# jeffreyyu0602/quantized-training

Hardware: AMD Instinct MI355X
Metric: quantized_elements_per_sec (higher is better)
Workload: dtype bf16; 1 GPU; llama-2-7b-shaped LLaMA (32 layers, hidden 4096, random init) WikiText-style window eval B=1 S=1024 stride 512, fake-quant activation=e4m3 weight=e4m3, --quantize_forward gemm (weights re-quantized every forward); route=eager, parallelism=dp1 (windows round-robin, metric all_gather only), launch=hipGraph replay, valid=True

## Files before the change

### quantized-training_amd/csrc/qt_attention_fp8.hip

```cpp
#include <hip/hip_runtime.h>
#include <stdint.h>
#include <stdlib.h>

#include "../../include/qt_hip.h"
#include "qt_device.h"
#include "qt_attention_split.h"
#include "qt_value_codes.h"
#include "qt_formats.h"

namespace {

typedef int v8i __attribute__((ext_vector_type(8)));

constexpr int kUnit = 127;

struct AttnArgs {
    const uint8_t *q8, *k8, *vt8;
    const uint16_t *mask;
    long msb, msh, msq;
    const int *row_live;
    long lsb, lsh, lsq;
    int mask_simple;
    uint16_t *out;
    int H, Sq, Sk;
// ... 18 lines not shown
        o = __builtin_amdgcn_cvt_scalef32_pk_fp8_bf16(o, __builtin_bit_cast(v2bf, p1), 1.0f, true);
    }
    return __builtin_bit_cast(uint32_t, o);
}

template <int F, int D, int MODE>
__device__ __forceinline__ void score_half(const uint8_t *blk, int t0, const v8i &qf, int f_lo, int f_hi, float scaling, float (*ev)[4], float &mx,
                                           const uint16_t *mrow, int key0, int my_live, int tiles) {
    uint2 m[4];
    if (MODE == 2) {
#pragma unroll
        for (int j = 0; j < 4; ++j) m[j] = *(const uint2 *)(mrow + key0 + j * 16);
    }
    u32x4 klo[4], khi[4];
#pragma unroll
    for (int j = 0; j < 4; ++j) {
        if (MODE == 1 && j >= tiles) continue;
        klo[j] = *(const u32x4 *)(blk + (t0 + j) * (16 * D) + f_lo);
        if (D == 128) khi[j] = *(const u32x4 *)(blk + (t0 + j) * (16 * D) + f_hi);
        else khi[j] = u32x4{0u, 0u, 0u, 0u};
    }
    v4f s[4];
#pragma unroll
    for (int j = 0; j < 4; ++j) {
        if (MODE == 1 && j >= tiles) continue;
        const v8i kf = {(int)klo[j].x, (int)klo[j].y, (int)klo[j].z, (int)klo[j].w, (int)khi[j].x, (int)khi[j].y, (int)khi[j].z, (int)khi[j].w};
        s[j] = __builtin_amdgcn_mfma_scale_f32_16x16x128_f8f6f4(kf, qf, v4f{0.f, 0.f, 0.f, 0.f}, F, F, 0, kUnit, 0, kUnit);
    }
    __builtin_amdgcn_sched_barrier(0);
#pragma unroll
    for (int j = 0; j < 4; ++j) {
        if (MODE == 1 && j >= tiles) {
            ev[j][0] = ev[j][1] = ev[j][2] = ev[j][3] = -INFINITY;
            continue;
        }
        uint32_t w0 = pack_bf16x2(s[j][0], s[j][1]), w1 = pack_bf16x2(s[j][2], s[j][3]);
        w0 = pack_bf16x2(bf_lo(w0) * scaling, bf_hi(w0) * scaling);
        w1 = pack_bf16x2(bf_lo(w1) * scaling, bf_hi(w1) * scaling);
        if (MODE == 2) {
            w0 = pack_bf16x2(bf_lo(w0) + bf_lo(m[j].x), bf_hi(w0) + bf_hi(m[j].x));
            w1 = pack_bf16x2(bf_lo(w1) + bf_lo(m[j].y), bf_hi(w1) + bf_hi(m[j].y));
        }
        float v[4] = {bf_lo(w0), bf_hi(w0), bf_lo(w1), bf_hi(w1)};
        if (MODE == 1) {
            const int left = my_live - (key0 + j * 16);
#pragma unroll
            for (int e = 0; e < 4; ++e) v[e] = (e < left || v[e] != v[e]) ? v[e] : -3.3895313892515355e38f;
        }
        ev[j][0] = v[0]; ev[j][1] = v[1]; ev[j][2] = v[2]; ev[j][3] = v[3];
        mx = max3(mx, v[0], v[1]);
        mx = max3(mx, v[2], v[3]);
    }
}

template <int F, int D, int MB>
__global__ __launch_bounds__(512, (MB == 4 && D == 64) ? 4 : 1) void attention_fp8_split_kernel(AttnArgs a) {
    constexpr int kBuf = kBlock * D;
    constexpr int kPieces = D / 32;
    extern __shared__ __attribute__((aligned(16))) uint8_t lds[];
    const int t = threadIdx.x, l = t & 63, w = __builtin_amdgcn_readfirstlane(t >> 6);
    const int r = l & 15, g = l >> 4, grp = w >> 2, wq = w & 3;
    const int bh = blockIdx.x, b = bh / a.H, h = bh % a.H;
    const int nkb = a.Sk / kBlock, nqb = (a.Sq + 63) / 64;
    const int qb = nqb - 1 - (int)blockIdx.y;
    const int q0 = qb * 64;
    const int qrow = q0 + wq * 16 + r, qc = min(qrow, a.Sq - 1);
    int nlive, wmax, wmin, my_live;
    split_row_extents(a, b, h, q0, qc, l, nkb, nlive, wmax, wmin, my_live);
    const int niter = (nlive + 1) / 2;
    const bool simple = a.mask && a.row_live && (a.mask_simple || (a.mask_irregular && *a.mask_irregular == 0)), full = a.mask && !simple;
    if (!simple) wmin = a.Sk;
    if (!simple && !a.row_live) wmax = a.Sk;
    const uint32_t l0 = lds_addr(lds);
    const uint8_t *kp[kPieces], *vp[kPieces];
#pragma unroll
    for (int i = 0; i < kPieces; ++i) {
        const int piece = (w * kPieces + i) % (D / 8);
        if (D == 128) {
            const int row = piece * 8 + (l >> 3), slot = l & 7, sw = ((slot ^ ((row >> 1) & 7)) << 4);
            kp[i] = a.k8 + ((long)bh * a.Sk + row) * D + sw;
        } else {
            const int r16 = l >> 2, row = piece * 16 + r16, sw = (((l & 3) ^ (((r16 >> 3) & 1) << 1)) << 4);
            kp[i] = a.k8 + ((long)bh * a.Sk + row) * D + sw;
        }
        const int vrow = piece * 8 + (l >> 3), vslot = l & 7, vsw = ((vslot ^ ((vrow >> 1) & 7)) << 4);
        vp[i] = a.vt8 + ((long)bh * D + vrow) * a.Sk + vsw;
    }
    auto issue_k = [&](int it) {
#pragma unroll
        for (int i = 0; i < kPieces; ++i) {
            const int piece = w * kPieces + i, kb = min(2 * it + piece / (D / 8), nkb - 1);
            dma16(kp[i] + (long)kb * kBuf, l0 + (2 * it) * kBuf + piece * 1024);
        }
    };
    auto issue_v = [&](int it) {
#pragma unroll
        for (int i = 0; i < kPieces; ++i) {
            const int piece = w * kPieces + i, kb = min(2 * it + piece / (D / 8), nkb - 1);
            dma16(vp[i] + (long)kb * kBlock, l0 + (2 * it) * kBuf + piece * 1024);
        }
    };
    auto wait_pair = [&](int it) {
        if (it + 1 < niter) asm volatile("s_waitcnt vmcnt(%0)" ::"n"(kPieces) : "memory");
        else asm volatile("s_waitcnt vmcnt(0)" ::: "memory");
        __builtin_amdgcn_s_barrier();
    };
// ... 68 lines not shown
    float sum = sum2[0] + sum2[1];
    sum += __shfl_xor(sum, 16, 64);
    sum += __shfl_xor(sum, 32, 64);
    if (g == 0) stat[128 + grp * 64 + wq * 16 + r] = sum;
    __syncthreads();
    const float inv = 1.0f / (stat[128 + wq * 16 + r] + stat[128 + 64 + wq * 16 + r]);
    constexpr int kDT = D / 16;
    v4f acc[kDT];
#pragma unroll
    for (int i = 0; i < kDT; ++i) acc[i] = v4f{0.f, 0.f, 0.f, 0.f};
#pragma unroll
    for (int it = 0; it < kIter; ++it) {
        if (it < niter) {
            wait_pair(it);
            if (it + 2 < niter) issue_v(it + 2);
            const bool live0 = tiles_of(2 * it) != 0, live1 = tiles_of(2 * it + 1) != 0;
            if (live0 | live1) {
                const uint8_t *blk = lds + (2 * it) * kBuf + f_v;
                u32x4 vlo[kDT], vhi[kDT];
#pragma unroll
                for (int dt = 0; dt < kDT / 2; ++dt) {
                    vlo[dt] = *(const u32x4 *)(blk + dt * 2048);
                    vhi[dt] = *(const u32x4 *)(blk + kBuf + dt * 2048);
                }
                uint32_t pd[8];
#pragma unroll
                for (int c = 0; c < 2; ++c) {
                    if (c == 0 ? live0 : live1) {
#pragma unroll
                        for (int j = 4 * c; j < 4 * c + 4; ++j) {
                            const float *v = e[it][j];
                            const uint32_t p0 = pack_bf16x2(v[0] * inv, v[1] * inv), p1 = pack_bf16x2(v[2] * inv, v[3] * inv);
                            pd[j] = prob_codes<F == 1>(p0, p1);
                        }
                    } else {
                        pd[4 * c] = pd[4 * c + 1] = pd[4 * c + 2] = pd[4 * c + 3] = 0;
                    }
                }
                const v8i pf = {(int)pd[0], (int)pd[1], (int)pd[2], (int)pd[3], (int)pd[4], (int)pd[5], (int)pd[6], (int)pd[7]};
#pragma unroll
                for (int dt = kDT / 2; dt < kDT; ++dt) {
                    vlo[dt] = *(const u32x4 *)(blk + dt * 2048);
                    vhi[dt] = *(const u32x4 *)(blk + kBuf + dt * 2048);
                }
                __builtin_amdgcn_sched_barrier(0);
#pragma unroll
                for (int dt = 0; dt < kDT; ++dt) {
                    const v8i vf = {(int)vlo[dt].x, (int)vlo[dt].y, (int)vlo[dt].z, (int)vlo[dt].w, (int)vhi[dt].x, (int)vhi[dt].y, (int)vhi[dt].z, (int)vhi[dt].w};
                    acc[dt] = __builtin_amdgcn_mfma_scale_f32_16x16x128_f8f6f4(vf, pf, acc[dt], F, F, 0, kUnit, 0, kUnit);
                }
            }
        }
    }
    const int prow = wq * 16 + r;
    split_park_partials(lds, acc, grp, prow, g);
    if (grp == 0 && qrow < a.Sq) {
#pragma unroll
        for (int dt = 0; dt < kDT; ++dt) {
            const float4 o = split_partial_sums<kDT>(lds, prow, dt, g);
            acc[dt][0] += o.x; acc[dt][1] += o.y; acc[dt][2] += o.z; acc[dt][3] += o.w;
        }
        const long o0 = (((long)b * a.Sq + qrow) * a.H + h) * D + 4 * g;
        uint16_t *orow = a.out + o0;
        if (a.out8) {
            const bool oe5 = a.out_fmt.p0 == 2;
#pragma unroll
            for (int dt = 0; dt < kDT; dt += 2) {
                uint32_t o[4] = {pack_bf16x2(acc[dt][0], acc[dt][1]), pack_bf16x2(acc[dt][2], acc[dt][3]),
                                 pack_bf16x2(acc[dt + 1][0], acc[dt + 1][1]), pack_bf16x2(acc[dt + 1][2], acc[dt + 1][3])};
                const uint2 codes = oe5 ? fq8_hw_vec8<true>(o, a.out_fmt) : fq8_hw_vec8<false>(o, a.out_fmt);
                *(uint2 *)(orow + dt * 16) = uint2{o[0], o[1]};
                *(uint2 *)(orow + dt * 16 + 16) = uint2{o[2], o[3]};
                *(uint32_t *)(a.out8 + o0 + dt * 16) = codes.x;
                *(uint32_t *)(a.out8 + o0 + dt * 16 + 16) = codes.y;
            }
        } else {
#pragma unroll
            for (int dt = 0; dt < kDT; ++dt)
                *(uint2 *)(orow + dt * 16) = uint2{pack_bf16x2(acc[dt][0], acc[dt][1]), pack_bf16x2(acc[dt][2], acc[dt][3])};
        }
    }
}

template <bool E5M2, int D>
__global__ __launch_bounds__(256) void value_codes_t_kernel(const uint16_t *v, uint8_t *vt8, int H, long Sk, long sb, long sh, long sk,
                                                            qt_format fmt) {
    __shared__ __attribute__((aligned(16))) uint8_t tile[D * kBlock];
    value_codes_block<E5M2, D>(tile, v, vt8, (int)blockIdx.x, (long)blockIdx.y, H, Sk, sb, sh, sk, fmt);
}

template <int F, int D, int MB>
int launch_split_mb(const AttnArgs &a, long BH, int nqb, hipStream_t st) {
    constexpr int kLds = MB * kBlock * D + 2 * 2 * 64 * 4;
    static_assert(MB * kBlock * D >= 64 * (D + 4) * 4, "the partial sums of the second wave group reuse the block buffers");
    if (qt_allow_lds<attention_fp8_split_kernel<F, D, MB>>(kLds)) return QT_ERR_BAD_ARG;
    attention_fp8_split_kernel<F, D, MB><<<dim3((unsigned)BH, (unsigned)nqb), 512, kLds, st>>>(a);
    return qt_launch_status();
}

template <int F, int D>
int launch_split(const AttnArgs &a, long BH, int nqb, hipStream_t st) {
    if constexpr (D == 64) {
        if (a.Sk <= 4 * kBlock) return launch_split_mb<F, D, 4>(a, BH, nqb, st);
    }
    return launch_split_mb<F, D, 8>(a, BH, nqb, st);
}

}

extern "C" {

int qt_value_codes_t(const uint16_t *v_dev, uint8_t *vt8_dev, long B, long H, long Sk, int head_dim, long stride_b, long stride_h, long stride_k,
                     const qt_format *fmt, void *stream) {
    if (B * H * Sk == 0) return QT_OK;
    const int f8 = qt_fp8_code(fmt);
    if (!v_dev || !vt8_dev || B < 0 || H < 1 || Sk < 0 || Sk % kBlock != 0 || B * H > 65535 || (head_dim != 64 && head_dim != 128) || !f8)
        return QT_ERR_BAD_ARG;
    const bool e5m2 = f8 == 2;
    if ((((uintptr_t)v_dev | (uintptr_t)vt8_dev) & 15u) || ((stride_b | stride_h | stride_k) & 7)) return QT_ERR_UNALIGNED;
    const dim3 grid((unsigned)(Sk / kBlock), (unsigned)(B * H));
    hipStream_t st = (hipStream_t)stream;
    if (head_dim == 128) {
        if (e5m2) value_codes_t_kernel<true, 128><<<grid, 256, 0, st>>>(v_dev, vt8_dev, (int)H, Sk, stride_b, stride_h, stride_k, *fmt);
        else value_codes_t_kernel<false, 128><<<grid, 256, 0, st>>>(v_dev, vt8_dev, (int)H, Sk, stride_b, stride_h, stride_k, *fmt);
    } else {
        if (e5m2) value_codes_t_kernel<true, 64><<<grid, 256, 0, st>>>(v_dev, vt8_dev, (int)H, Sk, stride_b, stride_h, stride_k, *fmt);
        else value_codes_t_kernel<false, 64><<<grid, 256, 0, st>>>(v_dev, vt8_dev, (int)H, Sk, stride_b, stride_h, stride_k, *fmt);
    }
    return qt_launch_status();
}

int qt_attention_fp8(const uint8_t *q8_dev, const uint8_t *k8_dev, const uint8_t *vt8_dev, int operand_format, const uint16_t *mask_dev,
                     long mask_sb, long mask_sh, long mask_sq, const int *row_live_dev, long live_sb, long live_sh, long live_sq,
                     int mask_is_simple, const int *mask_irregular_dev, uint16_t *out_dev, uint8_t *out8_dev, const qt_format *out_format, long B,
                     int H, int Sq, int Sk, int head_dim, float scaling, void *stream) {
    if (B * H * Sq == 0) return QT_OK;
    if (!q8_dev || !k8_dev || !vt8_dev || !out_dev || B < 0 || H < 1 || Sq < 1 || Sk < kBlock || Sk % kBlock != 0 || Sk > kBlock * kMaxBlocks ||
        B * H > 65535 || operand_format < 0 || operand_format > 1 || (head_dim != 64 && head_dim != 128))
        return QT_ERR_BAD_ARG;
    if ((((uintptr_t)q8_dev | (uintptr_t)k8_dev | (uintptr_t)vt8_dev) & 15u) || ((uintptr_t)out_dev & 7u) ||
        (mask_dev && ((((uintptr_t)mask_dev) & 7u) || ((mask_sb | mask_sh | mask_sq) & 3))))
        return QT_ERR_UNALIGNED;
    if (out8_dev && (!qt_fp8_code(out_format) || ((uintptr_t)out8_dev & 3u))) return QT_ERR_BAD_ARG;
    AttnArgs a{q8_dev, k8_dev, vt8_dev, mask_dev, mask_sb, mask_sh, mask_sq, row_live_dev, live_sb, live_sh, live_sq, mask_is_simple ? 1 : 0,
               out_dev, H, Sq, Sk, scaling, out8_dev, out8_dev ? *out_format : qt_format{}, mask_irregular_dev};
    const int nqb = (Sq + 63) / 64;
    hipStream_t st = (hipStream_t)stream;
    if (head_dim == 128) return operand_format == 0 ? launch_split<0, 128>(a, B * H, nqb, st) : launch_split<1, 128>(a, B * H, nqb, st);
    return operand_format == 0 ? launch_split<0, 64>(a, B * H, nqb, st) : launch_split<1, 64>(a, B * H, nqb, st);
}

}
```

### quantized-training_amd/quantized_training/fake_quantize.py

```python
import collections
import ctypes
import logging
from typing import Optional

import torch
from torch.ao.quantization import FakeQuantizeBase

from . import _native, handover, precomputed
from .quantizer.quantizer import QScheme

_PRE, _EXPECTED, _CHAIN_RESULT = precomputed.PRE.name, precomputed.EXPECTED.name, precomputed.CHAIN_RESULT.name

__all__ = [
    "FusedAmaxObsFakeQuantize",
    "_DerivedObserverOrFakeQuantize",
    "get_quantization_map",
]

logger = logging.getLogger(__name__)

class _Stats:
    elements = 0
    calls = 0

# ... 601 lines not shown
            "scale={}".format(
                self.fake_quant_enabled, self.observer_enabled, self.dtype, self.amax_history_len,
                self.quant_max, self.qscheme, self.ch_axis, self.block_size,
                self.force_scale_power_of_two, self.scale,
            )
        )

    def _move_to(self, device):
        if self.scale.device != device or self.amax_history.device != device:
            self.to(device)
        if self.qmap.device != device or (device.type == "cuda" and getattr(self.qmap, "_qt_dtype", None) is None):
            self.qmap = _table_for(self.dtype, device)
            if self.scale_qmap is not None:
                self.scale_qmap = _table_for(self.scale_dtype, device)

    def expect_prequantized(self, tensor, x8, replacement=None):
        precomputed.EXPECTED.leave(self, tensor, (x8, replacement))

    def producer_fusable(self) -> bool:
        return (self._quantize and not self._observe and self.qscheme is None and not self.is_per_channel
                and not self.record_histogram and self.outlier_threshold is None and self.fp8_exact())

    def forward(self, X: torch.Tensor) -> torch.Tensor:
        self.__dict__["_qt_calls"] = self.__dict__.get("_qt_calls", 0) + 1
        if "_qt_deferred" in self.__dict__:
            from . import train_fusions
            out = train_fusions.take_deferred(self, X)
            if out is not None:
                return out
        if _CHAIN_RESULT in self.__dict__ or "_qt_chain" in self.__dict__:
            from . import train_fusions
            out = train_fusions.take_member_result(self, X)
            if out is not None:
                return out
            chain = self.__dict__.get("_qt_chain")
            if chain is not None:
                out = train_fusions.run_chain(self, chain, X)
                if out is not None:
                    return out
        done_by = handover.done_by(X, unchecked=True)
        if done_by is self and handover.valid(X):
            _Stats.add(X.numel())
            if not self.__dict__.get("_qt_lazy_ok"):
                handover.materialize(X)
            return X
        also = handover.also_done(X)
        if also is not None:
            for fq, x8 in also:
                if fq is self:
                    _Stats.add(X.numel())
                    if handover.is_lazy(X) and not self.__dict__.get("_qt_lazy_ok"):
                        handover.materialize(X)
                    return handover.carry(X, x8, X)
        handover.materialize(X)
        if (done_by is not None and self._emit_fp8 and isinstance(done_by, FusedAmaxObsFakeQuantize)
                and handover.codes(X) is not None and X.is_cuda and X.dtype == torch.bfloat16 and X.is_contiguous()
                and not (torch.is_grad_enabled() and X.requires_grad) and self.producer_fusable() and done_by.producer_fusable()
                and done_by._qt_format.key() == self._qt_format.key()):
            self._move_to(X.device)
            _Stats.add(X.numel())
            x8 = FusedAmaxObsFakeQuantFunction.apply(X, False, True, self.qmap, self.amax_history, self.scale, self.amax_history_len,
                                                      self.quant_max, None, False, False, self._qt_format, "only")
            return handover.carry(X, x8, X)
        if _EXPECTED in self.__dict__:
            expect = precomputed.EXPECTED.take(self, X)
            if expect is not precomputed.MISS:
                x8, replacement = expect
                _Stats.add(X.numel())
                if replacement is not None:
                    out = handover.carry(replacement, x8.view(X.shape), X)
                    if handover.is_lazy(out) and not self.__dict__.get("_qt_lazy_ok"):
                        handover.materialize(out)
                    return out
                return handover.stamp(X, codes=x8)
        if _PRE in self.__dict__:
            out = precomputed.PRE.take(self, X)
            if out is not precomputed.MISS:
                _Stats.add(X.numel())
                if self._observe:
                    precomputed.take_preupdate(self.amax_history)
                return _PrecomputedFakeQuant.apply(X, out)
        self._move_to(X.device)

        if self.record_histogram:
            exp = torch.floor(torch.log2(torch.abs(X.detach().float())))
            self.histogram += torch.histc(exp, 254, min=-126, max=127)

        if self.outlier_threshold is not None:
            orig_X = X.clone()
            mask = torch.abs(X) < self.outlier_threshold
            X = torch.where(mask, X, torch.zeros_like(X))
            outlier_pct = mask.bitwise_not().sum().item() / X.numel()
            self.max_outlier_pct = max(outlier_pct, getattr(self, "max_outlier_pct", 0.0))

        if self.qscheme == QScheme.MICROSCALING:
            X = MXFakeQuantFunction.apply(X, self._quantize, self.scale, self.qmap, self.ch_axis, self.block_size,
                                          self.quant_max, self.force_scale_power_of_two, self.scale_qmap,
                                          self._qt_format)
            if self._quantize:
                _Stats.add(X.numel())
        elif self.qscheme == QScheme.GROUP_WISE_AFFINE:
            X = GroupWiseAffineFakeQuantFunction.apply(X, self._quantize, self.scale, self.zero_point, self.ch_axis,
                                                       self.block_size, self.quant_min, self.quant_max, self.scale_qmap)
        if self.qscheme in (QScheme.MICROSCALING, QScheme.GROUP_WISE_AFFINE):
            if self.outlier_threshold is not None:
                X = torch.where(mask, X, orig_X)
# ... 64 lines not shown
```

### quantized-training_amd/quantized_training/fused.py

```python
import collections
import ctypes

import torch

from . import _native, handover, planner_checks as pc, precomputed, switches
from .fake_quantize import STATS, FusedAmaxObsFakeQuantFunction, FusedAmaxObsFakeQuantize, _launch_format, _stream_ptr, launch_scale_update
from .quantizer.quantizer import QScheme

_IDENTITY = _native.QtFormat(_native.QT_FMT_IDENTITY, 0, 0, 0.0, 0.0)


def fused_gemm_enabled():
    return switches.on("QT_FUSED_GEMM")


def fp8_gemm_enabled():
    return switches.on("QT_FP8_GEMM")


def fq8_gemm_mode():
    return switches.mode("QT_FQ8_GEMM")


def fq8_gemm_enabled():
# ... 813 lines not shown

def _fp8_probs_times_v_or_none(L, st, scores, mask, msb, msh, msq, scaling, fq_p, fq_v, value, mask_owner=None):
    if (not switches.on("QT_FP8_ATTENTION") or not switches.on("QT_LT_GEMM") or not _LT["ok"]
            or fq_p is None or fq_v is None):
        return None
    if not (isinstance(fq_v, FusedAmaxObsFakeQuantize) and fq_p.producer_fusable() and fq_v.producer_fusable()):
        return None
    B, H, Q, C = scores.shape
    if value.dim() != 4 or value.shape[:3] != (B, H, C) or value.dtype != torch.bfloat16 or value.stride(-1) != 1:
        return None
    D = value.shape[-1]
    if D % 16 or C % 16 or any(s % 8 for s in value.stride()[:3]) or value.data_ptr() % 16 or B * H > 65535:
        return None
    if (B * H, Q, C, D) in _LT.setdefault("no_pv", set()):
        return None
    done = handover.done_by(value)
    v8 = handover.codes(value, unchecked=True)
    if not (done is fq_v and v8 is not None and value.is_contiguous()):
        v8u = torch.empty((B, H, C, D), dtype=torch.uint8, device=value.device)
        _native.check(L.qt_fake_quant_rows_bf16_fp8(value.data_ptr(), None, v8u.data_ptr(), B, H, C, D,
                                                    value.stride(0), value.stride(1), value.stride(2),
                                                    ctypes.byref(fq_v._qt_format), st), "qt_fake_quant_rows_bf16_fp8")
        v8 = handover.fp8_view(v8u, fq_v)
    p8u = torch.empty((B, H, Q, C), dtype=torch.uint8, device=scores.device)
    _native.check(L.qt_softmax_fq_bf16_fp8(scores.data_ptr(), mask.data_ptr() if mask is not None else None, None,
                                           p8u.data_ptr(), B, H, Q, C, msb, msh, msq, float(scaling),
                                           ctypes.byref(fq_p._qt_format), st), "qt_softmax_fq_bf16_fp8")
    p8 = handover.fp8_view(p8u, fq_p)
    out = lt_fp8_gemm(p8.view(B * H, Q, C), v8.view(B * H, C, D), None, b_is_kn=True)
    if out is None:
        _LT["no_pv"].add((B * H, Q, C, D))
        return None
    STATS.add(value.numel())
    STATS.add(scores.numel())
    return out.view(B, H, Q, D)


def _mask_strides(attention_mask, B, H, Q, C, device, align, no_grad=False):
    if attention_mask is None:
        return None, 0, 0, 0
    m = attention_mask[..., :C]
    if m.dtype != torch.bfloat16 or m.dim() != 4 or m.stride(-1) != 1 or m.device != device or (no_grad and m.requires_grad):
        return False
    if m.shape[0] not in (1, B) or m.shape[1] not in (1, H) or m.shape[2] not in (1, Q):
        return False
    sb = m.stride(0) if m.shape[0] == B and B > 1 else 0
    sh = m.stride(1) if m.shape[1] == H and H > 1 else 0
    sq = m.stride(2) if m.shape[2] == Q and Q > 1 else 0
    if (sb | sh | sq) % align != 0 or m.data_ptr() % (2 * align) != 0:
        return False
    return m, sb, sh, sq


def _attention_fp8_or_none(attn, query, key, value, attention_mask, scaling, fqs):
    fq_q, fq_k, fq_p, fq_v = fqs
    B, H, Q, D = query.shape
    C = key.shape[2]
    if D not in (64, 128) or C % 128 != 0 or C > 1024 or B * H > 65535 or value.dtype != torch.bfloat16 or value.stride(-1) != 1:
        return None
    if not all(isinstance(f, FusedAmaxObsFakeQuantize) and f.producer_fusable() for f in fqs):
        return None
    if len({f._qt_format.key() for f in fqs}) != 1 or any(s % 8 for s in value.stride()[:3]) or value.data_ptr() % 16:
        return None

    def handed(t, fq, rows):
        t8 = handover.codes(t)
        if t8 is None or handover.done_by(t) is not fq or not t8.is_contiguous() or tuple(t8.shape) != (B, H, rows, D):
            return None
        return t8

    def view_ok(t):
        return t.dtype == torch.bfloat16 and t.stride(-1) == 1 and not any(s % 8 for s in t.stride()[:3]) and t.data_ptr() % 16 == 0

    q8, k8 = handed(query, fq_q, Q), handed(key, fq_k, C)
    if (q8 is None and not view_ok(query)) or (k8 is None and not view_ok(key)):
        return None
    mk = _mask_strides(attention_mask, B, H, Q, C, query.device, 4)
    if mk is False:
        return None
    mask, msb, msh, msq = mk
    L = _native.lib()
    st = _stream_ptr(query)
    rl_ptr, lsb, lsh, lsq, irregular_ptr = None, 0, 0, 0, None
    if mask is not None:
        live = _mask_row_live(mask, attention_mask, B, H, Q, C, st)
        if live is not None:
            rl, lsb, lsh, lsq = live
            rl_ptr = rl.data_ptr()
            irregular_ptr = rl_ptr + 4 * (rl.numel() - 1)

    def codes(t, fq, t8, rows):
        if t8 is not None:
            fq.__dict__["_qt_calls"] = fq.__dict__.get("_qt_calls", 0) + 1
            STATS.add(t.numel())
            return t8
        t8 = torch.empty((B, H, rows, D), dtype=torch.uint8, device=t.device)
        _native.check(L.qt_fake_quant_rows_bf16_fp8(t.data_ptr(), None, t8.data_ptr(), B, H, rows, D, t.stride(0), t.stride(1), t.stride(2),
                                                    ctypes.byref(fq._qt_format), st), "qt_fake_quant_rows_bf16_fp8")
        STATS.add(t.numel())
        return t8

    def token_rows(t):
        b_, h_, s_, d_ = t.shape
        rs = t.stride(2)
        return rs if (t.stride(3) == 1 and t.stride(1) == d_ and t.stride(0) == s_ * rs and rs % 8 == 0 and rs >= h_ * d_) else None

    vt8 = None
    if (q8 is None and k8 is None and Q == C and key.shape[1] == H and value.shape[1] == H and token_rows(query) is not None
            and token_rows(key) is not None and switches.on("QT_ROPE_VALUE_LAUNCH")):
        q8 = torch.empty((B, H, Q, D), dtype=torch.uint8, device=query.device)
        k8 = torch.empty((B, H, C, D), dtype=torch.uint8, device=query.device)
        vt8 = torch.empty((B, H, D, C), dtype=torch.uint8, device=query.device)
        _native.check(L.qt_rope_fq_value(query.data_ptr(), key.data_ptr(), None, None, None, None, q8.data_ptr(), k8.data_ptr(), B, Q, H, H, D,
                                         token_rows(query), token_rows(key), ctypes.byref(fq_q._qt_format), ctypes.byref(fq_k._qt_format),
                                         value.data_ptr(), vt8.data_ptr(), value.stride(0), value.stride(1), value.stride(2),
                                         ctypes.byref(fq_v._qt_format), st), "qt_rope_fq_value")
        STATS.add(query.numel())
        STATS.add(key.numel())
    else:
        q8, k8 = codes(query, fq_q, q8, Q), codes(key, fq_k, k8, C)
    fmt = fq_v._qt_format
    early = attn.__dict__.pop("_qt_vt8", None)
    if vt8 is not None:
        pass
    elif early is not None and early[0] == value_key(value) and early[1] is fq_v:
        vt8 = early[2]
    else:
        vt8 = torch.empty((B, H, D, C), dtype=torch.uint8, device=query.device)
        _native.check(L.qt_value_codes_t(value.data_ptr(), vt8.data_ptr(), B, H, C, D, value.stride(0), value.stride(1), value.stride(2),
                                         ctypes.byref(fmt), st), "qt_value_codes_t")
    STATS.add(value.numel())
    STATS.add(B * H * Q * C)
    out = torch.empty((B, Q, H, D), dtype=torch.bfloat16, device=query.device)
    from .model_fusions import consumer_fq
    proj = getattr(attn, "o_proj", None) or attn.__dict__.get("_qt_out_proj")
    fq_o = consumer_fq(proj) if (proj is not None and switches.on("QT_FUSED_PRODUCER_FQ")) else None
    out8 = torch.empty((B, Q, H, D), dtype=torch.uint8, device=query.device) if fq_o is not None else None
    _native.check(L.qt_attention_fp8(q8.data_ptr(), k8.data_ptr(), vt8.data_ptr(), 1 if fmt.p0 == 2 else 0,
                                     mask.data_ptr() if mask is not None else None, msb, msh, msq, rl_ptr, lsb, lsh, lsq, 0, irregular_ptr,
                                     out.data_ptr(), out8.data_ptr() if out8 is not None else None,
                                     ctypes.byref(fq_o._qt_format) if fq_o is not None else None, B, H, Q, C, D, float(scaling), st),
                  "qt_attention_fp8")
    if fq_o is not None:
        fq_o.expect_prequantized(out, handover.fp8_view(out8, fq_o))
    return out


def fused_attention_or_none(attn, query, key, value, attention_mask, scaling, dropout):
    mode = switches.mode("QT_FUSED_ATTENTION")
    fp8_kernel = query.dim() == 4 and query.shape[-1] in (64, 128) and switches.on("QT_FP8_ATTENTION_KERNEL")
    if mode == "0" or (mode != "1" and query.shape[-1] != 64 and not fp8_kernel):
        return None
    if not (query.device.type == "cuda" and query.dtype == torch.bfloat16 and query.dim() == 4):
        return None
    if torch.is_grad_enabled() and (query.requires_grad or key.requires_grad or value.requires_grad):
        return None
    if dropout and attn.training:
        return None
    B, H, Q, D = query.shape
    C = key.shape[2]
    if D not in (64, 128) or C % 4 != 0 or key.shape != (B, H, C, D) or value.shape != (B, H, C, D) or B * H > 65535:
        return None
    for mod in (attn.attn_scaling, attn.softmax):
        if getattr(mod, "activation_pre_process", None) is not None or not pc.no_forward_hooks(mod):
            return None
    hq, hv = getattr(attn.qk_matmul, "activation_pre_process", None), getattr(attn.av_matmul, "activation_pre_process", None)
    if (hq is None) != (hv is None):
        return None
    fq_q = fq_k = fq_p = fq_v = None
    if not all(pc.quantize_hooks_only(mod, 0 if hq is None else 1) for mod in (attn.qk_matmul, attn.av_matmul)):
        return None
    if hq is not None:
        fqs_qk, fqs_av = (pc.holder_fqs(mod, "activation_pre_process", "0", "1", exact=False) for mod in (attn.qk_matmul, attn.av_matmul))
        if fqs_qk is None or fqs_av is None:
            return None
        fq_q, fq_k, fq_p, fq_v = *fqs_qk, *fqs_av
        if not all(pc.plain_per_tensor(f) for f in (fq_q, fq_k, fq_p, fq_v)):
            return None
    if fp8_kernel and fq_q is not None and switches.on("QT_FP8_ATTENTION"):
        out = _attention_fp8_or_none(attn, query, key, value, attention_mask, scaling, (fq_q, fq_k, fq_p, fq_v))
        if out is not None:
            return out
    table_p = (fq_p is not None and fq_p._quantize and fq_p._qt_format.kind == _native.QT_FMT_LUT)
    if mode != "1" and query.shape[-1] != 64 and not table_p:
        return None
    mk = _mask_strides(attention_mask, B, H, Q, C, query.device, 4)
    if mk is False:
        return None
    mask, msb, msh, msq = mk
    L = _native.lib()
    st = _stream_ptr(query)
    qq = (fq_q(query) if fq_q is not None else query).contiguous()
    kq = (fq_k(key) if fq_k is not None else key).contiguous()
    out = torch.empty((B, Q, H, D), dtype=torch.bfloat16, device=query.device)
    fmt, lut, scale_ptr, amax_ptr = _probs_fq_launch_args(fq_p, query.device, st, B * H * Q * C, drop_unit_scale=True)
# ... 76 lines not shown
```

### quantized-training_amd/quantized_training/handover.py

```python
import weakref

import torch

from . import switches


def valid(t):
    return getattr(t, "_qt_ver", None) == t._version


def tensor_key(t):
    return (t.data_ptr(), t._version, tuple(t.shape))


def fp8_view(t8, fmt):
    fmt = getattr(fmt, "_qt_format", fmt)
    return t8.view(torch.float8_e5m2 if fmt.p0 == 2 else torch.float8_e4m3fn)


def stamp(t, done_by=None, codes=None, also=None, origin=None, lazy=False, register=True):
    if done_by is not None:
        t._qt_fq_done_by = done_by
    if codes is not None:
        t._qt_fp8 = codes
# ... 23 lines not shown

def origin(t, unchecked=False):
    return _field(t, "_qt_origin", unchecked)


def also_done(t):
    return _field(t, "_qt_also_done")


def codes_of_transpose(t):
    return _field(t, "_qt_fp8_of_transpose")


def carry(X, x8, src):
    return stamp(X.view(src.shape), codes=x8, origin=tensor_key(src), lazy=is_lazy(X), register=False)


def transposed(key, key_t):
    if done_by(key) is not None:
        key_t._qt_fq_done_by = key._qt_fq_done_by
        if codes(key) is not None:
            key_t._qt_fp8_of_transpose = key._qt_fp8
        key_t._qt_ver = key._qt_ver
    return key_t


_LAZY = {}


def is_lazy(t):
    return t.__dict__.get("_qt_lazy", False)


def unwritten(shape=None, dtype=None, device=None, like=None, out=None):
    if out is None:
        out = torch.empty_like(like) if like is not None else torch.empty(shape, dtype=dtype, device=device)
    if switches.on("QT_LAZY_POISON"):
        out.fill_(float("nan"))
    return out


def mark_lazy(t):
    stamped = valid(t)
    unwritten(out=t)
    if stamped:
        t._qt_ver = t._version
    t._qt_lazy = True
    ptr = t.data_ptr()
    _LAZY[ptr] = weakref.ref(t)
    weakref.finalize(t, lambda p=ptr: _LAZY.pop(p, None) if (_LAZY.get(p) is not None and _LAZY[p]() is None) else None)
    return t


def materialize(t):
    if is_lazy(t):
        t.copy_(t._qt_fp8.to(t.dtype))
        t._qt_lazy = False
        t._qt_ver = t._version
        return
    if _LAZY:
        ref = _LAZY.get(t.data_ptr())
        base = ref() if ref is not None else None
        if (base is not None and base is not t and is_lazy(base) and base.device == t.device and base.dtype == t.dtype
                and base.numel() == t.numel() and t.is_contiguous()):
            stamped = valid(t)
            materialize(base)
            if stamped:
                t._qt_ver = t._version
```

### quantized-training_amd/quantized_training/model_fusions.py

```python
import ctypes
import logging

import torch

from . import _native, handover, planner_checks as pc, precomputed, switches
from .fake_quantize import FusedAmaxObsFakeQuantize, _stream_ptr

__all__ = ["apply_llama_fusions", "apply_bert_fusions", "rmsnorm", "silu_mul", "rope", "layernorm", "gelu"]


logger = logging.getLogger(__name__)
_DECLINED = set()


def _declined(what, why):
    if (what, why) not in _DECLINED:
        _DECLINED.add((what, why))
        logger.warning("quantized_training: %s keeps the Hugging Face code path: %s", what, why)


def _enabled():
    return switches.on("QT_FUSED_MODEL_OPS")


# ... 456 lines not shown
            return y
    return torch.nn.Embedding.forward(self, input)


def apply_bert_fusions(model):
    layers = []
    for mod in model.modules():
        att = getattr(mod, "attention", None)
        inner = getattr(att, "self", None) if att is not None else None
        if (inner is not None and all(hasattr(inner, n) for n in ("query", "key", "value"))
                and hasattr(getattr(att, "output", None), "LayerNorm") and hasattr(getattr(mod, "intermediate", None), "dense")
                and hasattr(getattr(mod, "output", None), "LayerNorm") and hasattr(mod.output, "dense")):
            layers.append(mod)
    problems = sorted({p for mod in layers for p in bert_layer_layout_problems(mod)})
    if problems:
        _declined("BERT-style launch fusions (LayerNorm / GELU forwards, q / k / v groups)", "; ".join(problems))
        return 0
    prev_norm = None
    for mod in model.modules():
        if type(mod).__name__.endswith("Embeddings") and isinstance(getattr(mod, "LayerNorm", None), torch.nn.LayerNorm):
            prev_norm = mod.LayerNorm
            if isinstance(getattr(mod, "dropout", None), torch.nn.Dropout):
                prev_norm.__dict__["_qt_dropout_after"] = mod.dropout
            if layers:
                for emb in mod.children():
                    if type(emb) is torch.nn.Embedding:
                        _bind(emb, _embedding_forward)
            break
    for i, mod in enumerate(layers):
        inner = mod.attention.self
        qkv = [inner.query, inner.key, inner.value]
        if all(hasattr(l, "weight_fake_quant") for l in qkv) and "_qt_sibling_group" not in inner.query.__dict__:
            from .fused import SiblingGroup
            group = SiblingGroup(qkv)
            for lin in qkv:
                lin.__dict__["_qt_sibling_group"] = group
        inner.__dict__["_qt_out_proj"] = mod.attention.output.dense
        if prev_norm is not None:
            prev_norm.__dict__["_qt_consumers"] = qkv
        mod.attention.output.LayerNorm.__dict__["_qt_consumers"] = [mod.intermediate.dense]
        mod.output.LayerNorm.__dict__.pop("_qt_consumers", None)
        mod.intermediate.__dict__["_qt_consumer"] = mod.output.dense
        _bind(mod.intermediate, _intermediate_forward)
        for norm in (prev_norm, mod.attention.output.LayerNorm, mod.output.LayerNorm):
            if type(norm) is torch.nn.LayerNorm:
                _bind(norm, _layernorm_forward)
        prev_norm = mod.output.LayerNorm
    return len(layers)


_CURRENT_ATTN = []


def _attn_enter(module, args, kwargs):
    _CURRENT_ATTN.append(module)
    module.__dict__["_qt_cacheless"] = kwargs.get("past_key_values") is None and kwargs.get("past_key_value") is None


def _attn_exit(module, args, kwargs, output):
    if _CURRENT_ATTN and _CURRENT_ATTN[-1] is module:
        _CURRENT_ATTN.pop()


def _qk_fqs(attn, table=False):
    mm = getattr(attn, "qk_matmul", None)
    fqs = pc.holder_fqs(mm, "activation_pre_process", "0", "1")
    if fqs is None or not pc.quantize_hooks_only(mm):
        return None
    fq_q, fq_k = fqs
    for f in fqs:
        if not isinstance(f, FusedAmaxObsFakeQuantize):
            return None
        if table:
            if not (f.stateless_map() and f._qt_format.kind == _native.QT_FMT_LUT) or not switches.on("QT_FUSED_PRODUCER_MAP"):
                return None
        elif not f.producer_fusable():
            return None
    if getattr(attn, "num_key_value_groups", 1) != 1:
        return None
    return fq_q, fq_k


def _rmsnorm_forward(self, hidden_states):
    pre = getattr(hidden_states, "_qt_prenormed", None)
    if pre is not None and pre[0] is self and pc.no_hooks(self):
        return pre[1]
    w = self.weight
    if (_eligible(hidden_states, w) and hidden_states.shape[-1] % 8 == 0 and hidden_states.shape[-1] <= 16384
            and hidden_states.numel() > 0 and w.is_contiguous()):
        fq = _norm_consumer_fq(self, allow_all=True, allow_map=True)
        if fq is not None:
            lazy = not (isinstance(fq, tuple) and fq and fq[0] == "map") and codes_only_ok(self.__dict__.get("_qt_consumers"), self)
            return rmsnorm_fq(hidden_states, w, self.variance_epsilon, fq, codes_only=lazy)
        return rmsnorm(hidden_states, w, self.variance_epsilon)
    return self._qt_hf_forward(hidden_states)


def _run_pre_hooks(mod, x):
    args = (x,)
    for hook_id, hook in mod._forward_pre_hooks.items():
        if hook_id in mod._forward_pre_hooks_with_kwargs:
            res = hook(mod, args, {})
            if res is not None:
                args = res[0]
        else:
            res = hook(mod, args)
            if res is not None:
                args = res if isinstance(res, tuple) else (res,)
    return args[0]


# ... 299 lines not shown
```

### quantized-training_amd/quantized_training/planner_checks.py

```python
from .fake_quantize import FusedAmaxObsFakeQuantize
from .quantizer.quantizer import QScheme


def no_hooks(mod):
    return not (mod._forward_hooks or mod._forward_pre_hooks or mod._backward_hooks or mod._backward_pre_hooks)


def no_forward_hooks(mod):
    return not (mod._forward_hooks or mod._forward_pre_hooks)


def no_output_hook(mod):
    return not mod._forward_hooks


def only_pre_hooks(mod):
    return not (mod._forward_hooks or mod._backward_hooks or mod._backward_pre_hooks)


def hook_counts(mod, forward_pre=None, forward=None, backward_pre=None, backward=None):
    for hooks, want in ((mod._forward_pre_hooks, forward_pre), (mod._forward_hooks, forward), (mod._backward_pre_hooks, backward_pre),
                        (mod._backward_hooks, backward)):
        if want is not None and (len(hooks) not in want if isinstance(want, tuple) else len(hooks) != want):
            return False
    return True


def quantize_hooks_only(mod, forward_pre=1, backward_pre=None):
    return hook_counts(mod, forward_pre, 0, backward_pre, None if backward_pre is None else 0)


def holder_fqs(mod, holder, *keys, exact=True):
    h = getattr(mod, holder, None)
    if h is None or (exact and len(h) != len(keys)) or any(k not in h for k in keys):
        return None
    return tuple(h[k] for k in keys)


def holder_fq(mod, holder, key="0", exact=False):
    h = getattr(mod, holder, None)
    return h[key] if h is not None and key in h and not (exact and len(h) != 1) else None


def linear_input_fq(linear):
    if not (len(linear._forward_pre_hooks) == 1 or linear.__dict__.get("_qt_prepared")):
        return None
    return holder_fq(linear, "activation_pre_process", exact=True)


def plain_per_tensor(fq):
    return (isinstance(fq, FusedAmaxObsFakeQuantize) and not fq.is_per_channel and fq.outlier_threshold is None and not fq.record_histogram
            and fq.qscheme not in (QScheme.MICROSCALING, QScheme.GROUP_WISE_AFFINE))
```

### quantized-training_amd/quantized_training/train_fusions.py

```python
import collections
import ctypes
import weakref

import torch

from . import _native, planner_checks as pc, precomputed, switches
from .handover import tensor_key, unwritten

__all__ = ["plan", "unplan", "enabled", "STATS"]


class _Counters:
    chains = 0
    members = 0
    colsums = 0
    colsum_fallbacks = 0
    misses = 0
    attention = 0
    fanins = 0
    deferred = 0
    embeddings = 0
    addlns = 0
    qkv_groups = 0
    qkv_forward_groups = 0
    missed = []

    @classmethod
    def reset(cls):
        cls.chains = cls.members = cls.colsums = cls.colsum_fallbacks = cls.misses = cls.attention = cls.fanins = cls.deferred = cls.embeddings = cls.addlns = cls.qkv_groups = cls.qkv_forward_groups = 0
        cls.missed = []


STATS = _Counters


DEBUG_BITS = {"chains": 1, "colsum": 2, "producers": 4, "attention": 8, "fanin": 16, "embedding": 32, "addln": 64, "qkvgemm": 128, "optimizer": 256,
              "pairgemm": 512, "qkvfwd": 1024}


def _on(name):
    return not (switches.mask("QT_TRAIN_DEBUG", DEBUG_BITS) & DEBUG_BITS[name])


def enabled():
    return _on("chains")


class Chain:

    def __init__(self, members, colsum=None, name=""):
        self.members = members
        self.colsum = colsum
        self.name = name


def put_colsum(g, gb):
    precomputed.COLSUM.put(g, gb)


_ATTN_ACTIVE = []


def _attn_enter(module, args, kwargs=None):
    _ATTN_ACTIVE.append(module)


def _attn_leave(module, args, output):
    from .modules.qat.linear import flush_forward
    if _ATTN_ACTIVE and _ATTN_ACTIVE[-1] is module:
        _ATTN_ACTIVE.pop()
    flush_forward()


def attention_block_active(owner_ref):
    owner = owner_ref() if owner_ref is not None else None
    return owner is not None and bool(_ATTN_ACTIVE) and _ATTN_ACTIVE[-1] is owner


def _mark_qkv_members(attn, lins):
    import weakref
    from .modules.qat.linear import Linear as QATLinear
    if not all(type(l) is QATLinear and pc.no_output_hook(l) and l.weight.shape == lins[0].weight.shape and (l.bias is None) == (lins[0].bias is None)
               for l in lins):
        return
    if not attn.__dict__.get("_qt_qkv_hooks", False):
        attn.register_forward_pre_hook(_attn_enter)
        attn.register_forward_hook(_attn_leave, always_call=True)
        attn.__dict__["_qt_qkv_hooks"] = True
    ref = weakref.ref(attn)
    for l in lins:
        l.__dict__["_qt_qkv_member"] = ref


def group_qkv_backward(lins, gys):
    from .modules.qat.linear import train_gemm_backward, train_gemm_group
    if not _on("qkvgemm") or len(lins) != 3 or len(gys) != 3:
        return False
    xs, ws, g2 = [], [], []
    for lin, gy in zip(lins, gys):
        xw = lin.__dict__.get("_qt_train_xw") if lin is not None else None
        if xw is None or gy is None:
            return False
        x, w = xw[0](), xw[1]()
        if x is None or w is None:
            return False
        if not (x.is_cuda and x.dtype == torch.bfloat16 and x.is_contiguous() and w.is_contiguous() and gy.is_contiguous()
                and gy.shape[:-1] == x.shape[:-1] and gy.shape[-1] == w.shape[0] and w.shape[1] == x.shape[-1]):
            return False
        xs.append(x.reshape(-1, x.shape[-1])); ws.append(w); g2.append(gy.reshape(-1, gy.shape[-1]))
    both = train_gemm_backward(g2, ws, xs, "q/k/v ")
    if both is not None:
        gxs, gws = both
    else:
        gxs = train_gemm_group(g2, ws, False, True, "dgrad q/k/v")
        if gxs is None:
            return False
        gws = train_gemm_group(g2, xs, True, True, "wgrad q/k/v")
        if gws is None:
            return False
# ... 875 lines not shown
```

Measured before the change: 897.4 billion elements/s.

## Stage attention epilogue through LDS and skip bf16 output when only codes needed

The attention kernel's epilogue now splits the cross-wave-group reduction so each group finishes half of the head dimension. It stages the finished bf16 values and fp8 codes in shared memory, then writes them out with coalesced 16-byte row stores. On the Python side, when the o_proj consumer only needs fp8 codes, the bf16 output buffer is left unwritten and lazily stamped. The fake-quantize path then reuses the precomputed codes without materializing it. This removes a full bf16 attention-output write and its later readback, at the cost of an extra barrier, stricter 16-byte alignment checks, and more complex lazy-tensor bookkeeping.

```diff
diff --git a/quantized-training_amd/csrc/qt_attention_fp8.hip b/quantized-training_amd/csrc/qt_attention_fp8.hip
--- a/quantized-training_amd/csrc/qt_attention_fp8.hip
+++ b/quantized-training_amd/csrc/qt_attention_fp8.hip
@@ -94,6 +94,11 @@
         mx = max3(mx, v[2], v[3]);
     }
 }
+
+template <int D> constexpr int kTilesAt = 2 * 64 * (D / 2 + 4) * 4;
+template <int D> constexpr int kValRow = 2 * D + 16;
+template <int D> constexpr int kCodeRow = D + 16;
+template <int D> constexpr int kEpilogueLds = kTilesAt<D> + 64 * (kValRow<D> + kCodeRow<D>);
 
 template <int F, int D, int MB>
 __global__ __launch_bounds__(512, (MB == 4 && D == 64) ? 4 : 1) void attention_fp8_split_kernel(AttnArgs a) {
@@ -268,33 +273,75 @@
             }
         }
     }
+    constexpr int kHalf = kDT / 2, kPartRow = 16 * kHalf + 4;
     const int prow = wq * 16 + r;
-    split_park_partials(lds, acc, grp, prow, g);
-    if (grp == 0 && qrow < a.Sq) {
-#pragma unroll
-        for (int dt = 0; dt < kDT; ++dt) {
-            const float4 o = split_partial_sums<kDT>(lds, prow, dt, g);
-            acc[dt][0] += o.x; acc[dt][1] += o.y; acc[dt][2] += o.z; acc[dt][3] += o.w;
-        }
-        const long o0 = (((long)b * a.Sq + qrow) * a.H + h) * D + 4 * g;
-        uint16_t *orow = a.out + o0;
+    float *part = (float *)lds;
+    uint8_t *tile_v = lds + kTilesAt<D>, *tile_c = tile_v + 64 * kValRow<D>;
+    v4f fin[kHalf];
+    __syncthreads();
+    {
+        float *mine = part + (grp * 64 + prow) * kPartRow + 4 * g;
+        if (grp == 0) {
+#pragma unroll
+            for (int j = 0; j < kHalf; ++j) {
+                *(float4 *)(mine + 16 * j) = float4{acc[kHalf + j][0], acc[kHalf + j][1], acc[kHalf + j][2], acc[kHalf + j][3]};
+                fin[j] = acc[j];
+            }
+        } else {
+#pragma unroll
+            for (int j = 0; j < kHalf; ++j) {
+                *(float4 *)(mine + 16 * j) = float4{acc[j][0], acc[j][1], acc[j][2], acc[j][3]};
+                fin[j] = acc[kHalf + j];
+            }
+        }
+    }
+    __syncthreads();
+    {
+        const float *theirs = part + ((1 - grp) * 64 + prow) * kPartRow + 4 * g;
+#pragma unroll
+        for (int j = 0; j < kHalf; ++j) {
+            const float4 o = *(const float4 *)(theirs + 16 * j);
+            fin[j][0] += o.x; fin[j][1] += o.y; fin[j][2] += o.z; fin[j][3] += o.w;
+        }
+    }
+    {
+        const int d0 = grp * (16 * kHalf) + 4 * g;
+        uint8_t *vrow = tile_v + prow * kValRow<D> + 2 * d0, *crow = tile_c + prow * kCodeRow<D> + d0;
         if (a.out8) {
             const bool oe5 = a.out_fmt.p0 == 2;
 #pragma unroll
-            for (int dt = 0; dt < kDT; dt += 2) {
-                uint32_t o[4] = {pack_bf16x2(acc[dt][0], acc[dt][1]), pack_bf16x2(acc[dt][2], acc[dt][3]),
-                                 pack_bf16x2(acc[dt + 1][0], acc[dt + 1][1]), pack_bf16x2(acc[dt + 1][2], acc[dt + 1][3])};
+            for (int j = 0; j < kHalf; j += 2) {
+                uint32_t o[4] = {pack_bf16x2(fin[j][0], fin[j][1]), pack_bf16x2(fin[j][2], fin[j][3]),
+                                 pack_bf16x2(fin[j + 1][0], fin[j + 1][1]), pack_bf16x2(fin[j + 1][2], fin[j + 1][3])};
                 const uint2 codes = oe5 ? fq8_hw_vec8<true>(o, a.out_fmt) : fq8_hw_vec8<false>(o, a.out_fmt);
-                *(uint2 *)(orow + dt * 16) = uint2{o[0], o[1]};
-                *(uint2 *)(orow + dt * 16 + 16) = uint2{o[2], o[3]};
-                *(uint32_t *)(a.out8 + o0 + dt * 16) = codes.x;
-                *(uint32_t *)(a.out8 + o0 + dt * 16 + 16) = codes.y;
+                if (a.out) {
+                    *(uint2 *)(vrow + j * 32) = uint2{o[0], o[1]};
+                    *(uint2 *)(vrow + j * 32 + 32) = uint2{o[2], o[3]};
+                }
+                *(uint32_t *)(crow + j * 16) = codes.x;
+                *(uint32_t *)(crow + j * 16 + 16) = codes.y;
             }
         } else {
 #pragma unroll
-            for (int dt = 0; dt < kDT; ++dt)
-                *(uint2 *)(orow + dt * 16) = uint2{pack_bf16x2(acc[dt][0], acc[dt][1]), pack_bf16x2(acc[dt][2], acc[dt][3])};
-        }
+            for (int j = 0; j < kHalf; ++j)
+                *(uint2 *)(vrow + j * 32) = uint2{pack_bf16x2(fin[j][0], fin[j][1]), pack_bf16x2(fin[j][2], fin[j][3])};
+        }
+    }
+    __syncthreads();
+    const int rows = min(64, a.Sq - q0);
+    const long orow0 = ((long)b * a.Sq + q0) * a.H + h;
+    if (a.out) {
+        constexpr int kCh = D / 8;
+#pragma unroll
+        for (int i = 0; i < 64 * kCh / 512; ++i) {
+            const int c = t + i * 512, row = c / kCh, ch = c % kCh;
+            if (row < rows) *(u32x4 *)((uint8_t *)a.out + (orow0 + (long)row * a.H) * (2 * D) + 16 * ch) = *(const u32x4 *)(tile_v + row * kValRow<D> + 16 * ch);
+        }
+    }
+    if (a.out8) {
+        constexpr int kCh = D / 16;
+        const int row = t / kCh, ch = t % kCh;
+        if (row < rows) *(u32x4 *)(a.out8 + (orow0 + (long)row * a.H) * D + 16 * ch) = *(const u32x4 *)(tile_c + row * kCodeRow<D> + 16 * ch);
     }
 }
 
@@ -308,7 +355,7 @@
 template <int F, int D, int MB>
 int launch_split_mb(const AttnArgs &a, long BH, int nqb, hipStream_t st) {
     constexpr int kLds = MB * kBlock * D + 2 * 2 * 64 * 4;
-    static_assert(MB * kBlock * D >= 64 * (D + 4) * 4, "the partial sums of the second wave group reuse the block buffers");
+    static_assert(MB * kBlock * D >= kEpilogueLds<D>, "the parked partial sums and the finished tile reuse the block buffers");
     if (qt_allow_lds<attention_fp8_split_kernel<F, D, MB>>(kLds)) return QT_ERR_BAD_ARG;
     attention_fp8_split_kernel<F, D, MB><<<dim3((unsigned)BH, (unsigned)nqb), 512, kLds, st>>>(a);
     return qt_launch_status();
@@ -351,13 +398,14 @@
                      int mask_is_simple, const int *mask_irregular_dev, uint16_t *out_dev, uint8_t *out8_dev, const qt_format *out_format, long B,
                      int H, int Sq, int Sk, int head_dim, float scaling, void *stream) {
     if (B * H * Sq == 0) return QT_OK;
-    if (!q8_dev || !k8_dev || !vt8_dev || !out_dev || B < 0 || H < 1 || Sq < 1 || Sk < kBlock || Sk % kBlock != 0 || Sk > kBlock * kMaxBlocks ||
+    if (!q8_dev || !k8_dev || !vt8_dev || (!out_dev && !out8_dev) || B < 0 || H < 1 || Sq < 1 || Sk < kBlock || Sk % kBlock != 0 || Sk > kBlock * kMaxBlocks ||
         B * H > 65535 || operand_format < 0 || operand_format > 1 || (head_dim != 64 && head_dim != 128))
         return QT_ERR_BAD_ARG;
-    if ((((uintptr_t)q8_dev | (uintptr_t)k8_dev | (uintptr_t)vt8_dev) & 15u) || ((uintptr_t)out_dev & 7u) ||
+    if ((((uintptr_t)q8_dev | (uintptr_t)k8_dev | (uintptr_t)vt8_dev) & 15u) || ((uintptr_t)out_dev & 15u) ||
         (mask_dev && ((((uintptr_t)mask_dev) & 7u) || ((mask_sb | mask_sh | mask_sq) & 3))))
         return QT_ERR_UNALIGNED;
-    if (out8_dev && (!qt_fp8_code(out_format) || ((uintptr_t)out8_dev & 3u))) return QT_ERR_BAD_ARG;
+    if (out8_dev && !qt_fp8_code(out_format)) return QT_ERR_BAD_ARG;
+    if ((uintptr_t)out8_dev & 15u) return QT_ERR_UNALIGNED;
     AttnArgs a{q8_dev, k8_dev, vt8_dev, mask_dev, mask_sb, mask_sh, mask_sq, row_live_dev, live_sb, live_sh, live_sq, mask_is_simple ? 1 : 0,
                out_dev, H, Sq, Sk, scaling, out8_dev, out8_dev ? *out_format : qt_format{}, mask_irregular_dev};
     const int nqb = (Sq + 63) / 64;
diff --git a/quantized-training_amd/quantized_training/fake_quantize.py b/quantized-training_amd/quantized_training/fake_quantize.py
--- a/quantized-training_amd/quantized_training/fake_quantize.py
+++ b/quantized-training_amd/quantized_training/fake_quantize.py
@@ -677,6 +677,12 @@
                     if handover.is_lazy(X) and not self.__dict__.get("_qt_lazy_ok"):
                         handover.materialize(X)
                     return handover.carry(X, x8, X)
+        rec = precomputed.EXPECTED.peek(self) if self.__dict__.get("_qt_lazy_ok") else None
+        if rec is not None and rec.payload[1] is None and handover.lazy_owner(X) is not None:
+            expect = precomputed.EXPECTED.take(self, X)
+            if expect is not precomputed.MISS:
+                _Stats.add(X.numel())
+                return handover.stamp(X, codes=expect[0].view(X.shape), lazy=True, register=False)
         handover.materialize(X)
         if (done_by is not None and self._emit_fp8 and isinstance(done_by, FusedAmaxObsFakeQuantize)
                 and handover.codes(X) is not None and X.is_cuda and X.dtype == torch.bfloat16 and X.is_contiguous()
diff --git a/quantized-training_amd/quantized_training/fused.py b/quantized-training_amd/quantized_training/fused.py
--- a/quantized-training_amd/quantized_training/fused.py
+++ b/quantized-training_amd/quantized_training/fused.py
@@ -889,6 +889,14 @@
     return m, sb, sh, sq
 
 
+def attention_output_plan(attn):
+    from .model_fusions import codes_only_ok, consumer_fq
+    own = getattr(attn, "o_proj", None)
+    proj = own or attn.__dict__.get("_qt_out_proj")
+    fq_o = consumer_fq(proj) if (proj is not None and switches.on("QT_FUSED_PRODUCER_FQ")) else None
+    return fq_o, fq_o is not None and own is not None and pc.no_foreign_hooks(attn) and codes_only_ok([proj])
+
+
 def _attention_fp8_or_none(attn, query, key, value, attention_mask, scaling, fqs):
     fq_q, fq_k, fq_p, fq_v = fqs
     B, H, Q, D = query.shape
@@ -968,16 +976,17 @@
                                          ctypes.byref(fmt), st), "qt_value_codes_t")
     STATS.add(value.numel())
     STATS.add(B * H * Q * C)
-    out = torch.empty((B, Q, H, D), dtype=torch.bfloat16, device=query.device)
-    from .model_fusions import consumer_fq
-    proj = getattr(attn, "o_proj", None) or attn.__dict__.get("_qt_out_proj")
-    fq_o = consumer_fq(proj) if (proj is not None and switches.on("QT_FUSED_PRODUCER_FQ")) else None
+    fq_o, codes_only = attention_output_plan(attn)
     out8 = torch.empty((B, Q, H, D), dtype=torch.uint8, device=query.device) if fq_o is not None else None
+    shape = (B, Q, H, D)
+    out = handover.unwritten(shape, torch.bfloat16, query.device) if codes_only else torch.empty(shape, dtype=torch.bfloat16, device=query.device)
     _native.check(L.qt_attention_fp8(q8.data_ptr(), k8.data_ptr(), vt8.data_ptr(), 1 if fmt.p0 == 2 else 0,
                                      mask.data_ptr() if mask is not None else None, msb, msh, msq, rl_ptr, lsb, lsh, lsq, 0, irregular_ptr,
-                                     out.data_ptr(), out8.data_ptr() if out8 is not None else None,
+                                     None if codes_only else out.data_ptr(), out8.data_ptr() if out8 is not None else None,
                                      ctypes.byref(fq_o._qt_format) if fq_o is not None else None, B, H, Q, C, D, float(scaling), st),
                   "qt_attention_fp8")
+    if codes_only:
+        handover.stamp(out, fq_o, handover.fp8_view(out8, fq_o), lazy=True)
     if fq_o is not None:
         fq_o.expect_prequantized(out, handover.fp8_view(out8, fq_o))
     return out
diff --git a/quantized-training_amd/quantized_training/handover.py b/quantized-training_amd/quantized_training/handover.py
--- a/quantized-training_amd/quantized_training/handover.py
+++ b/quantized-training_amd/quantized_training/handover.py
@@ -99,18 +99,26 @@
     return t
 
 
+def lazy_owner(t):
+    if not _LAZY:
+        return None
+    ref = _LAZY.get(t.data_ptr())
+    base = ref() if ref is not None else None
+    if (base is not None and base is not t and is_lazy(base) and base.device == t.device and base.dtype == t.dtype
+            and base.numel() == t.numel() and t.is_contiguous()):
+        return base
+    return None
+
+
 def materialize(t):
     if is_lazy(t):
         t.copy_(t._qt_fp8.to(t.dtype))
         t._qt_lazy = False
         t._qt_ver = t._version
         return
-    if _LAZY:
-        ref = _LAZY.get(t.data_ptr())
-        base = ref() if ref is not None else None
-        if (base is not None and base is not t and is_lazy(base) and base.device == t.device and base.dtype == t.dtype
-                and base.numel() == t.numel() and t.is_contiguous()):
-            stamped = valid(t)
-            materialize(base)
-            if stamped:
-                t._qt_ver = t._version
+    base = lazy_owner(t)
+    if base is not None:
+        stamped = valid(t)
+        materialize(base)
+        if stamped:
+            t._qt_ver = t._version
diff --git a/quantized-training_amd/quantized_training/model_fusions.py b/quantized-training_amd/quantized_training/model_fusions.py
--- a/quantized-training_amd/quantized_training/model_fusions.py
+++ b/quantized-training_amd/quantized_training/model_fusions.py
@@ -532,11 +532,13 @@
 _CURRENT_ATTN = []
 
 
+@pc.own_hook
 def _attn_enter(module, args, kwargs):
     _CURRENT_ATTN.append(module)
     module.__dict__["_qt_cacheless"] = kwargs.get("past_key_values") is None and kwargs.get("past_key_value") is None
 
 
+@pc.own_hook
 def _attn_exit(module, args, kwargs, output):
     if _CURRENT_ATTN and _CURRENT_ATTN[-1] is module:
         _CURRENT_ATTN.pop()
diff --git a/quantized-training_amd/quantized_training/planner_checks.py b/quantized-training_amd/quantized_training/planner_checks.py
--- a/quantized-training_amd/quantized_training/planner_checks.py
+++ b/quantized-training_amd/quantized_training/planner_checks.py
@@ -4,6 +4,16 @@
 
 def no_hooks(mod):
     return not (mod._forward_hooks or mod._forward_pre_hooks or mod._backward_hooks or mod._backward_pre_hooks)
+
+
+def own_hook(fn):
+    fn._qt_own_hook = True
+    return fn
+
+
+def no_foreign_hooks(mod):
+    return all(getattr(h, "_qt_own_hook", False)
+               for hooks in (mod._forward_hooks, mod._forward_pre_hooks, mod._backward_hooks, mod._backward_pre_hooks) for h in hooks.values())
 
 
 def no_forward_hooks(mod):
diff --git a/quantized-training_amd/quantized_training/train_fusions.py b/quantized-training_amd/quantized_training/train_fusions.py
--- a/quantized-training_amd/quantized_training/train_fusions.py
+++ b/quantized-training_amd/quantized_training/train_fusions.py
@@ -61,10 +61,12 @@
 _ATTN_ACTIVE = []
 
 
+@pc.own_hook
 def _attn_enter(module, args, kwargs=None):
     _ATTN_ACTIVE.append(module)
 
 
+@pc.own_hook
 def _attn_leave(module, args, output):
     from .modules.qat.linear import flush_forward
     if _ATTN_ACTIVE and _ATTN_ACTIVE[-1] is module:
```

Result: faster. 908.9 billion elements/s, median of 6 (+1.3%).
